# joe5saia/Hmc.jl

Hardware: NVIDIA B200
Metric: HMM state-steps/sec (windows x chains x T per Gibbs sweep) (higher is better)
Workload: dtype f32

## Files before the change

### hmc.jl_b200/csrc/hmcgpu.cu

```cuda
#include "../../include/hmcgpu.h"
#include "gibbs_wide_kernel.cuh"
#include "gibbs_scan_kernel.cuh"
#include "gibbs_seg_kernel.cuh"
#include "diagnostics.cuh"

#include <algorithm>
#include <chrono>
#include <condition_variable>
#include <cmath>
#include <cstdarg>
#include <cstdio>
#include <cstdlib>
#include <cstring>
#include <exception>
#include <map>
#include <memory>
#include <mutex>
#include <new>
#include <numeric>
#include <optional>
#include <string>
#include <thread>
#include <vector>

// ... 1083 lines not shown
    totS[slot] = w < 0 ? R(0) : (R)wi[w].totS;
    totQ[slot] = w < 0 ? R(0) : (R)wi[w].totQ;
    if (cntM) {
        totSm[slot] = w < 0 ? R(0) : (R)wi[w].totSm;
        totQm[slot] = w < 0 ? R(0) : (R)wi[w].totQm;
        totM[slot] = w < 0 ? 0 : (int)wi[w].totM;
    }
}

template <typename R>
__global__ void sigw_kernel(long long y_len, int S, const unsigned char* __restrict__ sig, double kappa,
                            unsigned char* __restrict__ mask_tm, R* __restrict__ out) {
    const long long i = blockIdx.x * (long long)blockDim.x + threadIdx.x;
    if (i >= y_len * S) return;
    const long long t = i / S;
    const int s = (int)(i % S);
    const bool f = sig && sig[(long long)s * y_len + t];
    if (mask_tm) mask_tm[i] = f ? 1 : 0;
    out[i] = f ? (R)(-1.0 / (1.0 + kappa)) : R(1);
}

template <typename R>
__global__ void __launch_bounds__(256) y_layout_kernel(long long y_len, int n_series, const double* __restrict__ in, R* __restrict__ yr) {
    __shared__ double tile[32][33];
    const long long s0 = (long long)blockIdx.x * 32, t0 = (long long)blockIdx.y * 32;
    const int tx = threadIdx.x & 31, ty = threadIdx.x >> 5;
#pragma unroll
    for (int j = ty; j < 32; j += 8) {
        const long long sidx = s0 + j, t = t0 + tx;
        if (sidx < n_series && t < y_len) tile[j][tx] = in[sidx * y_len + t];
    }
    __syncthreads();
#pragma unroll
    for (int j = ty; j < 32; j += 8) {
        const long long t = t0 + j, sidx = s0 + tx;
        if (sidx < n_series && t < y_len) yr[t * n_series + sidx] = (R)tile[tx][j];
    }
}

__global__ void summary_finish_kernel(long long n_elems, int F, double n, int has_loglik, const double* __restrict__ sum,
                                      const double* __restrict__ sumsq, double* __restrict__ mean, double* __restrict__ var) {
    const long long i = blockIdx.x * (long long)blockDim.x + threadIdx.x;
    if (i >= n_elems) return;
    const bool zero = !has_loglik && (int)(i % F) == F - 1;
    const double m = sum[i] / n;
    mean[i] = zero ? 0.0 : m;
    var[i] = zero ? 0.0 : fmax(0.0, __dsub_rn(sumsq[i] / n, __dmul_rn(m, m)));
}

template <typename R>
__global__ void yfut_kernel(int n_slots, int n_h, const int* __restrict__ slot_win, const double* __restrict__ yfut_w, R* __restrict__ out) {
    const int slot = blockIdx.x * blockDim.x + threadIdx.x;
    if (slot >= n_slots) return;
    const int w = slot_win[slot];
    for (int j = 0; j < n_h; ++j) out[(size_t)j * n_slots + slot] = w < 0 ? R(0) : (R)yfut_w[(size_t)w * n_h + j];
}

template <typename R>
__global__ void gather_draws_kernel(int K, int n_h, int n_slots, int chunk, int n_i, long long draw0, long long nrun, int n_chains,
                                    const int* __restrict__ slot_win, const int* __restrict__ slot_chain,
                                    const R* __restrict__ out, double* mu, double* sig2, double* A, double* pie, double* fc, double* ll) {
    const int i = blockIdx.y * blockDim.y + threadIdx.y;
    const int slot = blockIdx.x * blockDim.x + threadIdx.x;
    if (slot >= n_slots || i >= n_i) return;
    const int w = slot_win[slot];
    if (w < 0) return;
    const long long Rr = (long long)n_chains * nrun;
    const long long d = (long long)slot_chain[slot] * nrun + draw0 + i;
    const size_t cs = (size_t)chunk * n_slots;
    const R* o = out + (size_t)i * n_slots + slot;
    int f = 0;
    for (int k = 0; k < K; ++k, ++f) if (mu) mu[(size_t)w * Rr * K + (size_t)k * Rr + d] = (double)o[f * cs];
    for (int k = 0; k < K; ++k, ++f) if (sig2) sig2[(size_t)w * Rr * K + (size_t)k * Rr + d] = (double)o[f * cs];
    for (int k = 0; k < K * K; ++k, ++f) if (A) A[(size_t)w * Rr * K * K + (size_t)k * Rr + d] = (double)o[f * cs];
    for (int k = 0; k < K; ++k, ++f) if (pie) pie[(size_t)w * Rr * K + (size_t)k * Rr + d] = (double)o[f * cs];
    for (int k = 0; k < 2 * n_h; ++k, ++f) if (fc) fc[(size_t)w * Rr * 2 * n_h + (size_t)k * Rr + d] = (double)o[f * cs];
    if (ll) ll[(size_t)w * Rr + d] = (double)o[f * cs];
}

template <typename R>
__global__ void __launch_bounds__(128) summary_accum_kernel(int F, int n_slots, int chunk, int n_i, int n_chains,
                                                            const int* __restrict__ win_slot0, const R* __restrict__ out,
                                                            double* __restrict__ sum, double* __restrict__ sumsq) {
    __shared__ double sh[128];
    const int w = blockIdx.x, f = blockIdx.y;
    const int s0 = win_slot0[w];
    double a = 0.0, b = 0.0;
    const long long n = (long long)n_chains * n_i;
    for (long long j = threadIdx.x; j < n; j += blockDim.x) {
        const int cidx = (int)(j % n_chains), i = (int)(j / n_chains);
        const double v = (double)out[((size_t)f * chunk + i) * n_slots + s0 + cidx];
        a += v; b += v * v;
    }
    auto add = [](double x, double y2) { return x + y2; };
    a = block_reduce<double>(a, sh, add);
    b = block_reduce<double>(b, sh, add);
    if (threadIdx.x == 0) { sum[(size_t)w * F + f] += a; sumsq[(size_t)w * F + f] += b; }
}

template <typename R>
__global__ void tile_reduce_kernel(int K, int ncols, int n_chains, const int* __restrict__ win_slot0, const int* __restrict__ wT,
                                   const long long* __restrict__ warp_pi_off, const int* __restrict__ warp_T,
                                   const long long* __restrict__ win_off, R* __restrict__ acc_tile, double* __restrict__ win_sum) {
    const int w = blockIdx.x;
    const int N = wT[w];
    const int s0 = win_slot0[w];
    double* dst = win_sum + win_off[w] / K * ncols;
    for (int e = threadIdx.x; e < N * ncols; e += blockDim.x) {
        const int t = e / ncols, k = e % ncols;
        double acc = 0.0;
        for (int cidx = 0; cidx < n_chains; ++cidx) {
            const int slot = s0 + cidx;
            const int row = t + (warp_T[slot >> 5] - N);
            R* p = acc_tile + warp_pi_off[slot >> 5] / K * ncols + (size_t)(row * ncols + k) * 32 + (slot & 31);
            acc += (double)*p;
            *p = R(0);
        }
        dst[(size_t)k * N + t] += acc;
    }
}

struct SweepChoice {
    SweepKernel kernel = SweepKernel::thread;
    int seg_lanes = 0;
    int n_long = 0;
    int sweeps_per_launch = 16;
    int seg_threads = 128;
};

struct hmcgpu_plan {
    hmcgpu_ctx* ctx = nullptr;
    int K = 0, n_chains = 0, n_windows = 0, n_h = 0, precision = 32;
    long long burnin = 0, nrun = 0;
    unsigned flags = 0;
    unsigned long long seed = 0;
    int F = 0;
    std::vector<int> wT;
    std::vector<int> order;
    std::vector<long long> pib_off;
    long long pib_total = 0;
    long long state_steps = 0;
    int n_slots = 0, n_warps = 0, n_tasks = 0, chunk = 0, max_T = 0;
    GibbsArgs args{};
    DevBuf yr, wbase, wTd, wi, slot_win, slot_chain, T, ybase, warp_T, warp_pi_off, pi, pacc, facc, cnt, trans, Sd, Qd,
        events, cshift, xi, xi_user, chain_id, out, yfut_w, yfut, win_slot0, win_pib_off, totS, totQ, slot_pi_off;
    DevBuf sigmask, sigmask_tm, sigw, sbase, wsbase, wbase_init, X0, x0_off, cntM, Sm, Qm, totSm, totQm, totM;
    bool sig = false;
    Tuning tuning;
    SweepChoice sw;
    DevBuf yin;
    DevBuf warp_T_long, warp_pi_off_long;
    struct Group { int task0, stride, n_tasks, lanes; bool long_class; };
    std::vector<Group> groups;
    int n_groups = 1, n_bufs = 1;
    std::vector<cudaStream_t> gstreams;
    std::vector<cudaEvent_t> pool_events;
    std::vector<cudaEvent_t> timing_events;
    double launch_ms_sum = 0.0;
    DevBuf d_mu, d_sig2, d_A, d_pie, d_fc, d_ll, d_sum, d_sumsq, d_pibsum, d_fcsum;
    DevBuf dg_P, dg_S1, dg_head, dg_ring, dg_mean, dg_var, dg_gsum;
    DevBuf d_diag;
    unsigned long long seg_fallbacks[2] = {0, 0};
    cudaEvent_t ev0 = nullptr, ev1 = nullptr, evk0 = nullptr, evk1 = nullptr;
    double gpu_ms = 0.0, sweep_ms = 0.0;
    long long n_launches = 0, n_sweep_launches = 0, h2d = 0, d2h = 0;
    bool ran = false;
    ~hmcgpu_plan() {
        for (auto s2 : gstreams) cudaStreamDestroy(s2);
        for (auto e : pool_events) cudaEventDestroy(e);
        for (auto e : timing_events) cudaEventDestroy(e);
        if (ev0) cudaEventDestroy(ev0);
        if (ev1) cudaEventDestroy(ev1);
        if (evk0) cudaEventDestroy(evk0);
        if (evk1) cudaEventDestroy(evk1);
    }
};

static int validate_problem(hmcgpu_ctx* ctx, const hmcgpu_problem* p, const Tuning& t) {
    if (!ctx) return HMCGPU_ERR_ARG;
    if (!p) return fail(ctx, HMCGPU_ERR_ARG, "problem is NULL");
    if (!p->y || p->y_len < 2 || p->n_series < 1) return fail(ctx, HMCGPU_ERR_ARG, "empty series");
    if (p->n_windows < 1 || !p->win_start || !p->win_end) return fail(ctx, HMCGPU_ERR_ARG, "no windows");
    if (!k_supported(p->K)) return fail(ctx, HMCGPU_ERR_UNSUPPORTED, "K=%d not supported (2..32)", p->K);
    if (!k_thread_sweep(p->K, t) && (p->flags & HMCGPU_FLAG_SMOOTHED_MEAN))
        return fail(ctx, HMCGPU_ERR_UNSUPPORTED, "smoothed means are only implemented for K <= 8 (thread-per-chain kernels)");
    if (p->K > 4 && (p->flags & (HMCGPU_FLAG_SMOOTHED_MEAN | HMCGPU_FLAG_FILTERED_MEAN)) && p->n_h > 0) {
        const size_t b = p->precision / 8;
        const size_t need = (size_t)(p->K * b + 8 + 15) / 16 * 16 * p->K * 128 + b * 4 * 3 * 4 * p->K * 32 + b * (size_t)p->n_h * (p->K + 1) * 128;
        if (need > 200 * 1024)
            return fail(ctx, HMCGPU_ERR_UNSUPPORTED, "K=%d with %d in-sample forecast horizons needs %zu KB of shared memory per block: use fewer horizons", p->K, p->n_h, need / 1024);
    }
    if (p->flags & HMCGPU_FLAG_FILTERED_MEAN) {
        if (!k_thread_sweep(p->K, t)) return fail(ctx, HMCGPU_ERR_UNSUPPORTED, "filtered means are only implemented for K <= 8");
        if (p->flags & HMCGPU_FLAG_SMOOTHED_MEAN) return fail(ctx, HMCGPU_ERR_UNSUPPORTED, "HMCGPU_FLAG_FILTERED_MEAN and HMCGPU_FLAG_SMOOTHED_MEAN share their output arrays: one per call");
        if (p->is_signal || p->pi_row_back != 0) return fail(ctx, HMCGPU_ERR_UNSUPPORTED, "is_signal / pi_row_back cannot be combined with HMCGPU_FLAG_FILTERED_MEAN");
    }
    if (p->n_chains < 1) return fail(ctx, HMCGPU_ERR_ARG, "n_chains < 1");
    if ((long long)p->n_windows * p->n_chains > 0x7fffffffLL - 64)
        return fail(ctx, HMCGPU_ERR_UNSUPPORTED, "n_windows * n_chains = %lld exceeds 2^31 - 65 chains per call", (long long)p->n_windows * p->n_chains);
    if (p->burnin < 0 || p->nrun < 1) return fail(ctx, HMCGPU_ERR_ARG, "burnin < 0 or nrun < 1");
    if (p->burnin + p->nrun > 0xffffffffLL) return fail(ctx, HMCGPU_ERR_ARG, "more than 2^32 sweeps");
    if ((p->flags & HMCGPU_FLAG_DIAGNOSTICS) && p->nrun < 4) return fail(ctx, HMCGPU_ERR_ARG, "HMCGPU_FLAG_DIAGNOSTICS needs nrun >= 4 (two sequences of >= 2 draws per chain)");
    if (p->precision != 32 && p->precision != 64) return fail(ctx, HMCGPU_ERR_ARG, "precision must be 32 or 64");
    if (p->n_h < 0 || p->n_h > kMaxH || (p->n_h > 0 && !p->horizons)) return fail(ctx, HMCGPU_ERR_ARG, "0 <= n_h <= %d", kMaxH);
    if (p->is_signal || p->pi_row_back != 0) {
        if (!k_thread(p->K)) return fail(ctx, HMCGPU_ERR_UNSUPPORTED, "is_signal / pi_row_back are only implemented for K <= 4");
        if (p->flags & HMCGPU_FLAG_SMOOTHED_MEAN) return fail(ctx, HMCGPU_ERR_UNSUPPORTED, "is_signal / pi_row_back cannot be combined with HMCGPU_FLAG_SMOOTHED_MEAN");
        if (p->is_signal && !(p->kappa >= 0.0)) return fail(ctx, HMCGPU_ERR_ARG, "kappa must be >= 0 with is_signal");
        if (p->pi_row_back < 0) return fail(ctx, HMCGPU_ERR_ARG, "pi_row_back < 0");
    }
    for (int j = 0; j < p->n_h; ++j)
        if (p->horizons[j] < 0 || p->horizons[j] > kMaxHorizon) return fail(ctx, HMCGPU_ERR_ARG, "horizons must be in 0..%d", kMaxHorizon);
    for (int i = 0; i < p->K; ++i) {
        if ((p->alpha && !(p->alpha[i] > 0.0)) || (p->nu && !(p->nu[i] > 0.0)) || (p->beta0 && !(p->beta0[i] > 0.0)) || (p->beta && !(p->beta[i] > 0.0)))
            return fail(ctx, HMCGPU_ERR_ARG, "alpha, nu, beta0 and beta must be > 0 (state %d)", i + 1);
        if (p->xi && !std::isfinite(p->xi[i])) return fail(ctx, HMCGPU_ERR_ARG, "xi[%d] is not finite", i);
    }
    for (int w = 0; w < p->n_windows; ++w) {
        const long long wid = p->win_id ? (long long)p->win_id[w] : (long long)w;
        if (wid < 0 || (wid + 1) * (long long)p->n_chains > 0x100000000LL)
            return fail(ctx, HMCGPU_ERR_ARG, "window %d: win_id %lld with %d chains per window leaves the 32-bit chain-id range", w, wid, p->n_chains);
        const long long s = p->win_start[w], e = p->win_end[w];
        if (s < 1 || e > p->y_len || e - s + 1 < 2) return fail(ctx, HMCGPU_ERR_ARG, "window %d: [%lld,%lld] outside 1..%lld or shorter than 2", w, s, e, (long long)p->y_len);
        if (p->win_series && (p->win_series[w] < 0 || p->win_series[w] >= p->n_series)) return fail(ctx, HMCGPU_ERR_ARG, "window %d: bad series index", w);
        if (p->win_init_series && (p->win_init_series[w] < 0 || p->win_init_series[w] >= p->n_series)) return fail(ctx, HMCGPU_ERR_ARG, "window %d: bad init series index", w);
        if (p->pi_row_back >= e - s + 1) return fail(ctx, HMCGPU_ERR_ARG, "window %d: pi_row_back %d >= window length", w, p->pi_row_back);
    }
    if (p->X0) {
        size_t off = 0;
        for (int w = 0; w < p->n_windows; ++w) {
            const long long n = (long long)p->win_end[w] - p->win_start[w] + 1;
            for (long long i = 0; i < n; ++i)
                if (p->X0[off + i] < 1 || p->X0[off + i] > p->K) return fail(ctx, HMCGPU_ERR_ARG, "X0: state %lld of window %d is outside 1..%d", (long long)p->X0[off + i], w, p->K);
            off += (size_t)n;
        }
    }
    return 0;
}

static int scan_max_T_of(int precision, int K) { DISPATCH_K(K, return precision == 32 ? scan_max_T<float, KK>() : scan_max_T<double, KK>()); return 0; }
static long long seg_max_T_of(int K, int lanes) { DISPATCH_K(K, return seg_max_T<KK>(lanes)); return 0; }

static int choose_sweep(hmcgpu_ctx* ctx, const hmcgpu_problem* p, const std::vector<int>& wT, const std::vector<int>& order,
                        const Tuning& t, SweepChoice& c) {
    const int K = p->K, nw = p->n_windows, nc = p->n_chains, max_T = wT[order[0]];
    const bool sig = p->is_signal != nullptr || p->pi_row_back != 0;
    const bool acc_mean = p->flags & (HMCGPU_FLAG_SMOOTHED_MEAN | HMCGPU_FLAG_FILTERED_MEAN);
    const long long n_real = (long long)nw * nc;
    const long long full = (long long)ctx->sm_count * 16 * 32;
    c = SweepChoice{};
    if (!k_thread_sweep(K, t)) c.kernel = SweepKernel::lane;
// ... 213 lines not shown
    CU(ctx, pl->cnt.alloc((size_t)K * n_slots * sizeof(int)));
    CU(ctx, pl->trans.alloc((size_t)K * K * n_slots * sizeof(int)));
    CU(ctx, pl->Sd.alloc((size_t)K * n_slots * sizeof(R)));
    CU(ctx, pl->Qd.alloc((size_t)K * n_slots * sizeof(R)));
    CU(ctx, pl->events.alloc((size_t)n_slots * sizeof(int)));
    CU(ctx, pl->cshift.alloc((size_t)n_slots * sizeof(R)));
    CU(ctx, pl->xi.alloc((size_t)K * n_slots * sizeof(R)));
    CU(ctx, pl->totS.alloc((size_t)n_slots * sizeof(R)));
    CU(ctx, pl->totQ.alloc((size_t)n_slots * sizeof(R)));
    CU(ctx, pl->out.alloc(per_draw * (size_t)chunk * pl->n_bufs));
    CU(ctx, pl->yfut.alloc((size_t)std::max(1, p->n_h) * n_slots * sizeof(R)));
    const size_t Rr = (size_t)nc * p->nrun;
    if (p->flags & HMCGPU_FLAG_DRAWS) {
        CU(ctx, pl->d_mu.alloc((size_t)nw * Rr * K * sizeof(double)));
        CU(ctx, pl->d_sig2.alloc((size_t)nw * Rr * K * sizeof(double)));
        CU(ctx, pl->d_A.alloc((size_t)nw * Rr * K * K * sizeof(double)));
        CU(ctx, pl->d_pie.alloc((size_t)nw * Rr * K * sizeof(double)));
        if (p->n_h > 0) CU(ctx, pl->d_fc.alloc((size_t)nw * Rr * 2 * p->n_h * sizeof(double)));
        if (p->flags & HMCGPU_FLAG_LOGLIK) CU(ctx, pl->d_ll.alloc((size_t)nw * Rr * sizeof(double)));
    }
    if (p->flags & HMCGPU_FLAG_SUMMARY) {
        CU(ctx, pl->d_sum.alloc((size_t)nw * pl->F * sizeof(double)));
        CU(ctx, pl->d_sumsq.alloc((size_t)nw * pl->F * sizeof(double)));
    }
    if (p->flags & HMCGPU_FLAG_DIAGNOSTICS) {
        const size_t n_sf = (size_t)pl->F * n_slots, nwf = (size_t)nw * pl->F;
        CU(ctx, pl->dg_P.alloc(n_sf * kDiagLags * sizeof(double)));
        CU(ctx, pl->dg_S1.alloc(n_sf * sizeof(double)));
        CU(ctx, pl->dg_head.alloc(n_sf * kDiagLags * sizeof(R)));
        CU(ctx, pl->dg_ring.alloc(n_sf * kDiagLags * sizeof(R)));
        CU(ctx, pl->dg_mean.alloc(nwf * 2 * nc * sizeof(double)));
        CU(ctx, pl->dg_var.alloc(nwf * 2 * nc * sizeof(double)));
        CU(ctx, pl->dg_gsum.alloc(nwf * kDiagLags * sizeof(double)));
    }
    if (p->flags & kAccMean) {
        CU(ctx, pl->pacc.alloc((size_t)lay.pi_elems * sizeof(R)));
        if (p->n_h > 0) {
            CU(ctx, pl->facc.alloc((size_t)lay.pi_elems / K * p->n_h * sizeof(R)));
            CU(ctx, pl->d_fcsum.alloc((size_t)pib_total / K * p->n_h * sizeof(double)));
        }
        CU(ctx, pl->d_pibsum.alloc((size_t)pib_total * sizeof(double)));
    }
    const size_t smem = (size_t)pl->max_T;
    if (smem > 200 * 1024) return fail(ctx, HMCGPU_ERR_UNSUPPORTED, "window longer than %d observations", 200 * 1024);
    if (smem > 48 * 1024) CU(ctx, cudaFuncSetAttribute(window_init_kernel, cudaFuncAttributeMaxDynamicSharedMemorySize, (int)smem));
    window_init_kernel<<<nw, 256, smem, st>>>(K, yin.as<double>(), 1, pl->wbase.as<long long>(), pl->wbase_init.as<long long>(),
                                              pl->wTd.as<int>(), p->is_signal ? pl->sigmask_tm.as<unsigned char>() : nullptr,
                                              pl->wsbase.as<long long>(), sld, pl->X0.as<long long>(),
                                              pl->x0_off.as<long long>(), pl->wi.as<WinInit>());
    CU(ctx, cudaGetLastError());
    tr.sync_mark(st, "  tables, allocations, window statistics");
    yfut_kernel<R><<<grid_for(n_slots, 128), 128, 0, st>>>(n_slots, p->n_h, pl->slot_win.as<int>(), pl->yfut_w.as<double>(), pl->yfut.as<R>());
    CU(ctx, cudaGetLastError());

    GibbsArgs& a = pl->args;
    a.n_slots = n_slots; a.T = pl->T.as<int>(); a.ybase = pl->ybase.as<long long>(); a.yld = nser; a.y = pl->yr.p;
    a.warp_T = pl->warp_T.as<int>(); a.warp_pi_off = pl->warp_pi_off.as<long long>(); a.pi = pl->pi.p; a.pib_acc = pl->pacc.p; a.fc_acc = pl->facc.p;
    a.cnt = pl->cnt.as<int>(); a.trans = pl->trans.as<int>(); a.Sd = pl->Sd.p; a.Qd = pl->Qd.p; a.events = pl->events.as<int>();
    a.cshift = pl->cshift.p; a.xi = pl->xi.p; a.totS = pl->totS.p; a.totQ = pl->totQ.p; a.n_warps = n_warps;
    for (int i = 0; i < 32; ++i) {
        a.alpha[i] = (p->alpha && i < K) ? p->alpha[i] : 1.0;
        a.nu[i] = (p->nu && i < K) ? p->nu[i] : 1.0;
        a.beta0[i] = (p->beta0 && i < K) ? p->beta0[i] : 1.0;
        a.beta[i] = (p->beta && i < K) ? p->beta[i] : 2.0;
    }
    a.k0 = (unsigned)p->seed; a.k1 = (unsigned)(p->seed >> 32); a.chain_id = pl->chain_id.as<unsigned>();
    a.burnin = p->burnin; a.out = pl->out.p; a.chunk = pl->chunk; a.n_h = p->n_h;
    for (int j = 0; j < p->n_h; ++j) { a.h_sorted[j] = p->horizons[hs[j]]; a.h_slot[j] = hs[j]; }
    a.yfut = pl->yfut.p; a.flags = p->flags;
    a.sigw = pl->sigw.p; a.sbase = pl->sbase.as<long long>(); a.sld = sld; a.cntM = pl->cntM.as<int>(); a.Sm = pl->Sm.p; a.Qm = pl->Qm.p; a.totSm = pl->totSm.p; a.totQm = pl->totQm.p;
    a.totM = pl->totM.as<int>(); a.kappa = p->kappa; a.pi_back = p->pi_row_back;
    a.y_sm_elems = (y_in_smem<R>() && nser == 1 && K <= 4 && pl->sw.kernel == SweepKernel::thread && (size_t)p->y_len * sizeof(R) <= (size_t)kYSmemMaxBytes &&
                    pl->tuning.y_smem) ? (int)p->y_len : 0;
    a.all_signal = 0;
    if (p->is_signal) {
        const size_t nm = (size_t)p->y_len * sld;
        size_t ones = 0;
        for (size_t q = 0; q < nm; ++q) ones += p->is_signal[q] != 0;
        a.all_signal = ones == nm;
    }
    a.seg_warm = pl->tuning.seg_warm; a.seg_barriers = pl->tuning.seg_barriers;
    if (pl->sw.kernel == SweepKernel::seg) CU(ctx, pl->d_diag.alloc(2 * sizeof(unsigned long long)));
    a.diag = pl->d_diag.as<unsigned long long>();
    for (int g = 0; g < pl->n_groups; ++g) {
        cudaStream_t s2;
        CU(ctx, cudaStreamCreateWithFlags(&s2, cudaStreamNonBlocking));
        pl->gstreams.push_back(s2);
    }
    CU(ctx, cudaEventCreate(&pl->ev0)); CU(ctx, cudaEventCreate(&pl->ev1));
    CU(ctx, cudaEventCreate(&pl->evk0)); CU(ctx, cudaEventCreate(&pl->evk1));
    tr.mark("  tables, allocations, init");
    CU(ctx, cudaStreamSynchronize(st));
    tr.mark("  stream drained");
    pl->yin.release();
    return HMCGPU_OK;
}

template <typename R, int K>
static int plan_run_t(hmcgpu_plan* pl) {
    hmcgpu_ctx* ctx = pl->ctx;
    cudaStream_t st = ctx->stream;
    const int ns = pl->n_slots, G = pl->n_groups;
    const int L = pl->sw.sweeps_per_launch;
    const int Kr = pl->K;
    pl->n_launches = 0; pl->n_sweep_launches = 0; pl->sweep_ms = 0.0;
    size_t ev_used = 0;
    auto new_event = [&](cudaEvent_t* e) -> cudaError_t {
        if (ev_used == pl->pool_events.size()) {
            cudaEvent_t x;
            cudaError_t rc = cudaEventCreateWithFlags(&x, cudaEventDisableTiming);
            if (rc != cudaSuccess) return rc;
            pl->pool_events.push_back(x);
        }
        *e = pl->pool_events[ev_used++];
        return cudaSuccess;
    };
    CU(ctx, cudaEventRecord(pl->ev0, st));
    chain_init_kernel<R><<<grid_for(ns, 128), 128, 0, st>>>(Kr, ns, pl->slot_win.as<int>(), pl->wi.as<WinInit>(),
                                                             pl->xi_user.as<double>(), pl->cnt.as<int>(), pl->trans.as<int>(),
                                                             pl->Sd.as<R>(), pl->Qd.as<R>(), pl->cshift.as<R>(), pl->xi.as<R>(),
                                                             pl->totS.as<R>(), pl->totQ.as<R>(), pl->events.as<int>(),
                                                             pl->cntM.as<int>(), pl->Sm.as<R>(), pl->Qm.as<R>(), pl->totSm.as<R>(),
                                                             pl->totQm.as<R>(), pl->totM.as<int>());
    CU(ctx, cudaGetLastError());
    ++pl->n_launches;
    if (pl->d_diag.p) CU(ctx, cudaMemsetAsync(pl->d_diag.p, 0, 2 * sizeof(unsigned long long), st));
    if (pl->d_sum.p) { CU(ctx, cudaMemsetAsync(pl->d_sum.p, 0, pl->d_sum.bytes, st)); CU(ctx, cudaMemsetAsync(pl->d_sumsq.p, 0, pl->d_sumsq.bytes, st)); }
    if (pl->pacc.p) { CU(ctx, cudaMemsetAsync(pl->pacc.p, 0, pl->pacc.bytes, st)); CU(ctx, cudaMemsetAsync(pl->d_pibsum.p, 0, pl->d_pibsum.bytes, st)); }
    if (pl->facc.p) { CU(ctx, cudaMemsetAsync(pl->facc.p, 0, pl->facc.bytes, st)); CU(ctx, cudaMemsetAsync(pl->d_fcsum.p, 0, pl->d_fcsum.bytes, st)); }
    cudaEvent_t ev_init;
    CU(ctx, new_event(&ev_init));
    CU(ctx, cudaEventRecord(ev_init, st));
    CU(ctx, cudaEventRecord(pl->evk0, st));
    for (int g = 0; g < G; ++g) CU(ctx, cudaStreamWaitEvent(pl->gstreams[g], ev_init, 0));
    size_t tev_used = 0;
    auto timing_event = [&](cudaEvent_t* e) -> cudaError_t {
        if (tev_used == pl->timing_events.size()) {
            cudaEvent_t x;
            cudaError_t rc = cudaEventCreate(&x);
            if (rc != cudaSuccess) return rc;
            pl->timing_events.push_back(x);
        }
        *e = pl->timing_events[tev_used++];
        return cudaSuccess;
    };
    std::vector<cudaEvent_t> gend(G, nullptr);
    for (int g = 0; g < G; ++g) CU(ctx, timing_event(&gend[g]));
    std::vector<std::pair<cudaEvent_t, cudaEvent_t>> launch_pairs;

    const GibbsLaunch cfg{pl->flags, pl->max_T, ctx->sm_count, pl->n_h, pl->sig};
    const long long S = pl->burnin + pl->nrun;
    const long long n_chunks = (pl->nrun + pl->chunk - 1) / pl->chunk;
    const size_t buf_elems = (size_t)pl->F * pl->chunk * ns;
    std::vector<long long> next(G, 0);
    std::vector<cudaEvent_t> post_done(n_chunks, nullptr);
    std::vector<std::vector<cudaEvent_t>> chunk_done(n_chunks, std::vector<cudaEvent_t>(G, nullptr));
    long long posted = 0;
    auto enqueue_post = [&](long long k) -> int {
        for (int g = 0; g < G; ++g) CU(ctx, cudaStreamWaitEvent(st, chunk_done[k][g], 0));
        const long long d0 = k * pl->chunk;
        const int n = (int)std::min<long long>(pl->chunk, pl->nrun - d0);
        const R* buf = pl->out.as<R>() + (size_t)(k % pl->n_bufs) * buf_elems;
        if (pl->flags & HMCGPU_FLAG_DRAWS) {
            dim3 blk(32, 8), grd(grid_for(ns, 32), grid_for(n, 8));
            gather_draws_kernel<R><<<grd, blk, 0, st>>>(Kr, pl->n_h, ns, pl->chunk, n, d0, pl->nrun, pl->n_chains, pl->slot_win.as<int>(),
                                                         pl->slot_chain.as<int>(), buf, pl->d_mu.as<double>(), pl->d_sig2.as<double>(),
                                                         pl->d_A.as<double>(), pl->d_pie.as<double>(), pl->d_fc.as<double>(), pl->d_ll.as<double>());
            CU(ctx, cudaGetLastError());
            ++pl->n_launches;
        }
        if (pl->flags & HMCGPU_FLAG_SUMMARY) {
            dim3 grd(pl->n_windows, pl->F);
            summary_accum_kernel<R><<<grd, 128, 0, st>>>(pl->F, ns, pl->chunk, n, pl->n_chains, pl->win_slot0.as<int>(), buf,
                                                         pl->d_sum.as<double>(), pl->d_sumsq.as<double>());
            CU(ctx, cudaGetLastError());
            ++pl->n_launches;
        }
        if (pl->flags & HMCGPU_FLAG_DIAGNOSTICS) {
            const long long nh = pl->nrun / 2, h2 = pl->nrun - nh;
            const int Fd = (pl->flags & HMCGPU_FLAG_LOGLIK) ? pl->F : pl->F - 1;
            const DiagState<R> ds{pl->dg_P.as<double>(), pl->dg_S1.as<double>(), pl->dg_head.as<R>(), pl->dg_ring.as<R>(), (long long)pl->F * ns};
            auto sequence = [&](long long lo, long long hi, long long seq0, long long seq_end, int half) -> int {
                if (lo >= hi) return 0;
                diag_accum_kernel<R><<<dim3(ns / 32, Fd), dim3(32, 32), 0, st>>>(ns, pl->chunk, (int)(lo - d0), (int)(hi - lo), lo - seq0, buf, ds);
                CU(ctx, cudaGetLastError());
                ++pl->n_launches;
                if (hi == seq_end) {
                    diag_half_kernel<R><<<dim3(pl->n_windows, Fd), kDiagLags, 0, st>>>(pl->F, ns, pl->n_chains, nh, half, pl->win_slot0.as<int>(), ds,
                                                                                       pl->dg_mean.as<double>(), pl->dg_var.as<double>(), pl->dg_gsum.as<double>());
                    CU(ctx, cudaGetLastError());
                    ++pl->n_launches;
                }
                return 0;
            };
            TRY(sequence(d0, std::min<long long>(d0 + n, nh), 0, nh, 0));
            TRY(sequence(std::max(d0, h2), d0 + n, h2, pl->nrun, 1));
        }
        if (pl->flags & (HMCGPU_FLAG_SMOOTHED_MEAN | HMCGPU_FLAG_FILTERED_MEAN)) {
            tile_reduce_kernel<R><<<pl->n_windows, 256, 0, st>>>(Kr, Kr, pl->n_chains, pl->win_slot0.as<int>(), pl->wTd.as<int>(),
                                                                 pl->warp_pi_off.as<long long>(), pl->warp_T.as<int>(), pl->win_pib_off.as<long long>(),
                                                                 pl->pacc.as<R>(), pl->d_pibsum.as<double>());
            CU(ctx, cudaGetLastError());
            ++pl->n_launches;
            if (pl->facc.p) {
                tile_reduce_kernel<R><<<pl->n_windows, 256, 0, st>>>(Kr, pl->n_h, pl->n_chains, pl->win_slot0.as<int>(), pl->wTd.as<int>(),
                                                                     pl->warp_pi_off.as<long long>(), pl->warp_T.as<int>(), pl->win_pib_off.as<long long>(),
                                                                     pl->facc.as<R>(), pl->d_fcsum.as<double>());
                CU(ctx, cudaGetLastError());
                ++pl->n_launches;
            }
        }
        CU(ctx, new_event(&post_done[k]));
        CU(ctx, cudaEventRecord(post_done[k], st));
        return 0;
    };
    GibbsArgs a = pl->args;
    auto enqueue_one = [&](const int g, const long long round) -> int {
            const long long s0 = next[g];
            if (s0 >= S) return 1;
            if (s0 >= pl->burnin && (s0 - pl->burnin) % pl->chunk == 0) {
                const long long k0 = (s0 - pl->burnin) / pl->chunk;
                if (k0 >= pl->n_bufs && post_done[k0 - pl->n_bufs] == nullptr) return 1;
            }
            long long n = (round == 0 && G > 1) ? std::max<long long>(1, (long long)L * (g + 1) / G) : L;
            long long limit = S;
            if (s0 < pl->burnin) limit = pl->burnin;
            else limit = pl->burnin + std::min<long long>(pl->nrun, ((s0 - pl->burnin) / pl->chunk + 1) * pl->chunk);
            n = std::min(n, limit - s0);
            cudaStream_t gs = pl->gstreams[g];
            long long k = -1;
            if (s0 >= pl->burnin) {
                k = (s0 - pl->burnin) / pl->chunk;
                if ((s0 - pl->burnin) % pl->chunk == 0 && k >= pl->n_bufs) CU(ctx, cudaStreamWaitEvent(gs, post_done[k - pl->n_bufs], 0));
                a.draw0 = k * pl->chunk;
                a.out = pl->out.as<R>() + (size_t)(k % pl->n_bufs) * buf_elems;
            } else {
                a.draw0 = 0;
                a.out = pl->out.p;
            }
            a.sweep0 = s0; a.n_sweeps = (int)n;
            const hmcgpu_plan::Group& grp = pl->groups[g];
            a.task0 = grp.task0; a.task_stride = grp.stride; a.n_tasks = grp.n_tasks;
            a.warp_T = grp.long_class ? pl->warp_T_long.as<int>() : pl->warp_T.as<int>();
            a.warp_pi_off = grp.long_class ? pl->warp_pi_off_long.as<long long>() : pl->warp_pi_off.as<long long>();
            cudaEvent_t lt0 = nullptr, lt1 = nullptr;
            if (pl->tuning.launch_timing) { CU(ctx, timing_event(&lt0)); CU(ctx, timing_event(&lt1)); CU(ctx, cudaEventRecord(lt0, gs)); }
            if constexpr (K == 0) {
                CU(ctx, (launch_gibbs_wide<R>(cfg, a, pl->K, pl->slot_pi_off.as<long long>(), gs)));
            } else if constexpr (K <= 4) {
                switch (pl->sw.kernel) {
                    case SweepKernel::scan: CU(ctx, (launch_gibbs_scan<R, K>(cfg, a, gs))); break;
                    case SweepKernel::seg: CU(ctx, (launch_gibbs_seg<R, K>(cfg, a, grp.lanes, pl->sw.seg_threads, gs))); break;
                    default: CU(ctx, (launch_gibbs<R, K>(cfg, a, gs)));
                }
            } else {
                CU(ctx, (launch_gibbs<R, K>(cfg, a, gs)));
            }
            if (pl->tuning.launch_timing) { CU(ctx, cudaEventRecord(lt1, gs)); launch_pairs.emplace_back(lt0, lt1); }
            ++pl->n_launches; ++pl->n_sweep_launches;
            next[g] = s0 + n;
            if (next[g] >= S) CU(ctx, cudaEventRecord(gend[g], gs));
            if (k >= 0 && next[g] == pl->burnin + std::min<long long>(pl->nrun, (k + 1) * pl->chunk)) {
                CU(ctx, new_event(&chunk_done[k][g]));
                CU(ctx, cudaEventRecord(chunk_done[k][g], gs));
            }
            while (posted < n_chunks) {
                bool ready = true;
                for (int g2 = 0; g2 < G; ++g2) ready = ready && chunk_done[posted][g2] != nullptr;
                if (!ready) break;
                TRY(enqueue_post(posted));
                ++posted;
            }
            return 0;
    };
    PhaseTrace trr;
    bool more = true;
    for (long long round = 0; more; ++round) {
        more = false;
        std::vector<int> gorder(G);
        std::iota(gorder.begin(), gorder.end(), 0);
        std::stable_sort(gorder.begin(), gorder.end(), [&](int x, int y2) { return next[x] < next[y2]; });
        for (int g : gorder) {
            if (next[g] >= S) continue;
            more = true;
            const int rc = enqueue_one(g, round);
            if (rc < 0) return rc;
        }
    }
    CU(ctx, cudaEventRecord(pl->ev1, st));
    trr.mark("    launches enqueued");
    CU(ctx, cudaEventSynchronize(pl->ev1));
    trr.mark("    device drained");
    for (int g = 0; g < G; ++g) CU(ctx, cudaStreamSynchronize(pl->gstreams[g]));
    float ms = 0.f;
    CU(ctx, cudaEventElapsedTime(&ms, pl->ev0, pl->ev1));
    pl->gpu_ms = ms;
    pl->sweep_ms = 0.0;
    for (int g = 0; g < G; ++g) {
        float t = 0.f;
        CU(ctx, cudaEventElapsedTime(&t, pl->evk0, gend[g]));
        pl->sweep_ms = std::max(pl->sweep_ms, (double)t);
    }
    pl->launch_ms_sum = 0.0;
    for (auto& pr : launch_pairs) {
        float t = 0.f;
        CU(ctx, cudaEventElapsedTime(&t, pr.first, pr.second));
        pl->launch_ms_sum += t;
    }
    if (pl->d_diag.p) {
        CU(ctx, cudaMemcpy(pl->seg_fallbacks, pl->d_diag.p, 2 * sizeof(unsigned long long), cudaMemcpyDeviceToHost));
        if (pl->tuning.verbose) {
            const double cs = (double)pl->n_windows * pl->n_chains * (double)S;
            if (pl->sw.n_long) fprintf(stderr, "[hmcgpu] segment kernel: the %d longest of %d windows with 8 lanes per chain\n", pl->sw.n_long, pl->n_windows);
            fprintf(stderr, "[hmcgpu] segment kernel (%d lanes per chain, warm-up %d): %llu of %.0f chain-sweeps used the exact entering vectors; "
                            "%.2f speculative groups of 4 steps per chain-sweep\n",
                    pl->sw.seg_lanes, pl->args.seg_warm, pl->seg_fallbacks[0], cs, (double)pl->seg_fallbacks[1] / cs);
        }
    }
    pl->ran = true;
    return HMCGPU_OK;
}

static int plan_create_impl(hmcgpu_ctx* ctx, const hmcgpu_problem* p, hmcgpu_plan** out) {
    const Tuning t = read_tuning();
    TRY(validate_problem(ctx, p, t));
    CU(ctx, cudaSetDevice(ctx->device));
    tl_pool = ctx->pool;
    std::unique_ptr<hmcgpu_plan> pl(new hmcgpu_plan());
    pl->ctx = ctx;
    pl->tuning = t;
    int rc = (p->precision == 32) ? plan_build<float>(pl.get(), p) : plan_build<double>(pl.get(), p);
    if (rc != 0) {
        cudaStreamSynchronize(ctx->stream);
        cudaGetLastError();
        return rc;
    }
    *out = pl.release();
    return HMCGPU_OK;
}

extern "C" int hmcgpu_plan_create(hmcgpu_ctx* ctx, const hmcgpu_problem* p, hmcgpu_plan** out) {
    if (!out) return fail(ctx, HMCGPU_ERR_ARG, "out is NULL");
    *out = nullptr;
    GUARD(ctx, plan_create_impl(ctx, p, out));
}

static int plan_run_impl(hmcgpu_plan* pl) {
    hmcgpu_ctx* ctx = pl->ctx;
    CU(ctx, cudaSetDevice(ctx->device));
    int rc = HMCGPU_ERR_UNSUPPORTED;
    DISPATCH_RUN(pl, rc);
    return rc;
}

extern "C" int hmcgpu_plan_run(hmcgpu_plan* pl) {
    if (!pl) return HMCGPU_ERR_ARG;
    GUARD(pl->ctx, plan_run_impl(pl));
}

static int plan_fetch_impl(hmcgpu_plan* pl, hmcgpu_result* r);
extern "C" int hmcgpu_plan_fetch(hmcgpu_plan* pl, hmcgpu_result* r) {
    if (!pl || !r) return HMCGPU_ERR_ARG;
    GUARD(pl->ctx, plan_fetch_impl(pl, r));
}

static int plan_fetch_impl(hmcgpu_plan* pl, hmcgpu_result* r) {
    hmcgpu_ctx* ctx = pl->ctx;
    if (!pl->ran) return fail(ctx, HMCGPU_ERR_ARG, "plan_fetch before plan_run");
    CU(ctx, cudaSetDevice(ctx->device));
    cudaStream_t st = ctx->stream;
    const int K = pl->K, nw = pl->n_windows;
    const size_t Rr = (size_t)pl->n_chains * pl->nrun;
    long long d2h = 0;
    auto down = [&](void* host, const DevBuf& b, size_t bytes) -> cudaError_t {
        if (!host || !b.p) return cudaSuccess;
        d2h += (long long)bytes;
        return cudaMemcpyAsync(host, b.p, bytes, cudaMemcpyDeviceToHost, st);
    };
    if ((r->mu || r->sigma2 || r->A || r->pi_end || r->forecasts || r->loglik) && !(pl->flags & HMCGPU_FLAG_DRAWS))
        return fail(ctx, HMCGPU_ERR_ARG, "per-draw outputs requested without HMCGPU_FLAG_DRAWS");
    if ((r->summary_mean || r->summary_var) && !(pl->flags & HMCGPU_FLAG_SUMMARY))
        return fail(ctx, HMCGPU_ERR_ARG, "summary requested without HMCGPU_FLAG_SUMMARY");
    if ((r->pib_mean || r->insample_forecast_mean) && !(pl->flags & (HMCGPU_FLAG_SMOOTHED_MEAN | HMCGPU_FLAG_FILTERED_MEAN)))
        return fail(ctx, HMCGPU_ERR_ARG, "pib_mean / insample_forecast_mean requested without HMCGPU_FLAG_SMOOTHED_MEAN or HMCGPU_FLAG_FILTERED_MEAN");
    if (r->loglik && !(pl->flags & HMCGPU_FLAG_LOGLIK)) return fail(ctx, HMCGPU_ERR_ARG, "loglik requested without HMCGPU_FLAG_LOGLIK");
    const bool diag = (pl->flags & HMCGPU_FLAG_DIAGNOSTICS) && (r->rhat || r->ess || r->ess_lag);
    CU(ctx, down(r->mu, pl->d_mu, nw * Rr * K * sizeof(double)));
    CU(ctx, down(r->sigma2, pl->d_sig2, nw * Rr * K * sizeof(double)));
    CU(ctx, down(r->A, pl->d_A, nw * Rr * K * K * sizeof(double)));
    CU(ctx, down(r->pi_end, pl->d_pie, nw * Rr * K * sizeof(double)));
    CU(ctx, down(r->forecasts, pl->d_fc, nw * Rr * 2 * pl->n_h * sizeof(double)));
    CU(ctx, down(r->loglik, pl->d_ll, nw * Rr * sizeof(double)));
    std::vector<double> pibsum, fcsum;
    std::vector<int> ev(pl->n_slots);
    DevBuf d_mean, d_var;
    if (r->summary_mean || r->summary_var) {
        const long long ne = (long long)nw * pl->F;
        CU(ctx, d_mean.alloc((size_t)ne * sizeof(double)));
        CU(ctx, d_var.alloc((size_t)ne * sizeof(double)));
        summary_finish_kernel<<<grid_for(ne, 256), 256, 0, st>>>(ne, pl->F, (double)Rr, (pl->flags & HMCGPU_FLAG_LOGLIK) ? 1 : 0,
                                                                 pl->d_sum.as<double>(), pl->d_sumsq.as<double>(), d_mean.as<double>(), d_var.as<double>());
        CU(ctx, cudaGetLastError());
        CU(ctx, down(r->summary_mean, d_mean, (size_t)ne * sizeof(double)));
        CU(ctx, down(r->summary_var, d_var, (size_t)ne * sizeof(double)));
    }
    DevBuf d_rhat, d_ess, d_lag;
    if (diag) {
        const long long ne = (long long)nw * pl->F;
        CU(ctx, d_rhat.alloc((size_t)ne * sizeof(double)));
        CU(ctx, d_ess.alloc((size_t)ne * sizeof(double)));
        CU(ctx, d_lag.alloc((size_t)ne * sizeof(int)));
        diag_finish_kernel<<<grid_for(ne, 128), 128, 0, st>>>(ne, pl->F, pl->n_chains, pl->nrun / 2, (pl->flags & HMCGPU_FLAG_LOGLIK) ? 1 : 0,
                                                              pl->dg_mean.as<double>(), pl->dg_var.as<double>(), pl->dg_gsum.as<double>(),
                                                              d_rhat.as<double>(), d_ess.as<double>(), d_lag.as<int>());
        CU(ctx, cudaGetLastError());
        CU(ctx, down(r->rhat, d_rhat, (size_t)ne * sizeof(double)));
        CU(ctx, down(r->ess, d_ess, (size_t)ne * sizeof(double)));
        CU(ctx, down(r->ess_lag, d_lag, (size_t)ne * sizeof(int)));
    }
    if (r->pib_mean) { pibsum.resize((size_t)pl->pib_total); CU(ctx, down(pibsum.data(), pl->d_pibsum, pibsum.size() * sizeof(double))); }
    if (r->insample_forecast_mean && pl->d_fcsum.p) {
        fcsum.resize((size_t)pl->pib_total / K * pl->n_h);
        CU(ctx, down(fcsum.data(), pl->d_fcsum, fcsum.size() * sizeof(double)));
    }
    CU(ctx, down(ev.data(), pl->events, ev.size() * sizeof(int)));
    CU(ctx, cudaStreamSynchronize(st));
    const double n = (double)Rr;
    for (size_t i = 0; i < pibsum.size(); ++i) r->pib_mean[i] = pibsum[i] / n;
    for (size_t i = 0; i < fcsum.size(); ++i) r->insample_forecast_mean[i] = fcsum[i] / n;
    std::vector<int> slot_win(pl->n_slots), slot_chain(pl->n_slots);
    int bad = 0;
    for (int j = 0; j < nw; ++j) {
        const int w = pl->order[j];
        for (int c = 0; c < pl->n_chains; ++c) {
            const int e = ev[(size_t)j * pl->n_chains + c];
            if (r->status) r->status[(size_t)w * pl->n_chains + c] = e;
            bad += e != 0;
        }
    }
    r->gpu_ms = pl->gpu_ms; r->sweep_kernel_ms = pl->sweep_ms; r->n_launches = pl->n_launches;
    r->n_sweep_launches = pl->n_sweep_launches; r->h2d_bytes = pl->h2d; r->d2h_bytes = d2h; r->state_steps = pl->state_steps;
    r->sweep_launch_ms_sum = pl->launch_ms_sum;
    r->sweep_kernel = (int32_t)pl->sw.kernel;
    r->n_tasks = pl->n_tasks;
    return bad;
}

extern "C" void hmcgpu_plan_destroy(hmcgpu_plan* pl) {
    if (!pl) return;
    cudaSetDevice(pl->ctx->device);
    cudaStreamSynchronize(pl->ctx->stream);
    for (auto s2 : pl->gstreams) cudaStreamSynchronize(s2);
    delete pl;
}

extern "C" int hmcgpu_estimate(hmcgpu_ctx* ctx, const hmcgpu_problem* p, hmcgpu_result* r) {
    if (!r) return fail(ctx, HMCGPU_ERR_ARG, "result is NULL");
    hmcgpu_plan* pl = nullptr;
    PhaseTrace tr;
    TRY(hmcgpu_plan_create(ctx, p, &pl));
    tr.mark("plan_create (upload, init)");
    int rc = hmcgpu_plan_run(pl);
    tr.mark("plan_run (all sweeps)");
    if (rc == 0) rc = hmcgpu_plan_fetch(pl, r);
    tr.mark("plan_fetch (download)");
    hmcgpu_plan_destroy(pl);
    tr.mark("plan_destroy");
    return rc;
}

static int estimate_multi_impl(const int* devices, int n_dev, const hmcgpu_problem* p, hmcgpu_result* r);
extern "C" int hmcgpu_estimate_multi(const int* devices, int n_dev, const hmcgpu_problem* p, hmcgpu_result* r) {
    if (!devices || n_dev < 1 || !p || !r) return fail(nullptr, HMCGPU_ERR_ARG, "bad arguments");
    GUARD(nullptr, estimate_multi_impl(devices, n_dev, p, r));
}

static int estimate_multi_impl(const int* devices, int n_dev, const hmcgpu_problem* p, hmcgpu_result* r) {
    if (p->n_windows < 1 || !p->win_start || !p->win_end) return fail(nullptr, HMCGPU_ERR_ARG, "no windows");
    const int nw = p->n_windows, K = p->K, nh = p->n_h;
    std::vector<int> ord(nw);
    std::iota(ord.begin(), ord.end(), 0);
    auto Tw = [&](int w) { return p->win_end[w] - p->win_start[w] + 1; };
    std::stable_sort(ord.begin(), ord.end(), [&](int a, int b) { return Tw(a) > Tw(b); });
    std::vector<std::vector<int>> shard(n_dev);
    std::vector<long long> load(n_dev, 0);
    for (int w : ord) {
        const int d = (int)(std::min_element(load.begin(), load.end()) - load.begin());
        shard[d].push_back(w);
        load[d] += Tw(w);
    }
    const size_t Rr = (size_t)p->n_chains * p->nrun;
    const int F = 3 * K + K * K + 2 * nh + 1;
    std::vector<long long> pib_off(nw);
    long long acc = 0;
    for (int w = 0; w < nw; ++w) { pib_off[w] = acc; acc += (long long)Tw(w) * K; }
    std::vector<int> rcs(n_dev, 0);
    std::vector<std::string> errs(n_dev);
    std::vector<hmcgpu_result> parts(n_dev);
    std::vector<std::thread> th;
    for (int d = 0; d < n_dev; ++d) {
        th.emplace_back([&, d]() {
          hmcgpu_ctx* ctx = nullptr;
          try {
            const std::vector<int>& ws = shard[d];
            const int n = (int)ws.size();
            memset(&parts[d], 0, sizeof(hmcgpu_result));
            if (n == 0) return;
            int rc = hmcgpu_ctx_create(devices[d], &ctx);
            if (rc != 0) { rcs[d] = rc; errs[d] = hmcgpu_last_error(nullptr); return; }
            std::vector<int32_t> ser(n), iser(n), st(n), en(n);
            std::vector<int64_t> id(n), x0;
            size_t pibn = 0;
            for (int j = 0; j < n; ++j) {
                const int w = ws[j];
                ser[j] = p->win_series ? p->win_series[w] : 0; st[j] = p->win_start[w]; en[j] = p->win_end[w];
                iser[j] = p->win_init_series ? p->win_init_series[w] : ser[j];
                id[j] = p->win_id ? p->win_id[w] : w;
                pibn += (size_t)Tw(w) * K;
                if (p->X0) x0.insert(x0.end(), p->X0 + pib_off[w] / K, p->X0 + pib_off[w] / K + Tw(w));
            }
            hmcgpu_problem q = *p;
            q.n_windows = n; q.win_series = ser.data(); q.win_start = st.data(); q.win_end = en.data(); q.win_id = id.data();
            if (p->win_init_series) q.win_init_series = iser.data();
            if (p->X0) q.X0 = x0.data();
            std::vector<double> mu, s2, A, pe, fc, ll, sm, sv, pb, ifc, rh, es;
            std::vector<int32_t> status, el;
            const bool diag = (p->flags & HMCGPU_FLAG_DIAGNOSTICS) != 0;
            hmcgpu_result& o = parts[d];
            if (r->mu) { mu.resize(n * Rr * K); o.mu = mu.data(); }
            if (r->sigma2) { s2.resize(n * Rr * K); o.sigma2 = s2.data(); }
            if (r->A) { A.resize(n * Rr * K * K); o.A = A.data(); }
            if (r->pi_end) { pe.resize(n * Rr * K); o.pi_end = pe.data(); }
            if (r->forecasts) { fc.resize(n * Rr * 2 * nh); o.forecasts = fc.data(); }
            if (r->loglik) { ll.resize(n * Rr); o.loglik = ll.data(); }
            if (r->summary_mean) { sm.resize((size_t)n * F); o.summary_mean = sm.data(); }
// ... 55 lines not shown
```

Baseline: 227.4 billion.

## Run post-processing on low-priority stream and batch summary accumulation loads

Moves all per-chunk post-processing kernels (draw gather, summary, diagnostics, tile reduce) from the main context stream to a dedicated low-priority stream, and gives the Gibbs sweep group streams high priority. This lets post-processing overlap with sweeps instead of serializing on the main stream. The summary accumulation kernel is also rewritten to replace per-element div/mod indexing with incremental offsets and software-pipelined batched loads. The end-of-run event now waits on the last post event, which assumes n_chunks > 0 and that its event is non-null.

```diff
diff --git a/hmc.jl_b200/csrc/hmcgpu.cu b/hmc.jl_b200/csrc/hmcgpu.cu
--- a/hmc.jl_b200/csrc/hmcgpu.cu
+++ b/hmc.jl_b200/csrc/hmcgpu.cu
@@ -1189,15 +1189,46 @@
 __global__ void __launch_bounds__(128) summary_accum_kernel(int F, int n_slots, int chunk, int n_i, int n_chains,
                                                             const int* __restrict__ win_slot0, const R* __restrict__ out,
                                                             double* __restrict__ sum, double* __restrict__ sumsq) {
+    constexpr int kBatch = 8;
     __shared__ double sh[128];
     const int w = blockIdx.x, f = blockIdx.y;
-    const int s0 = win_slot0[w];
+    const int t = threadIdx.x, nt = blockDim.x;
+    const int n = n_chains * n_i;
+    const int cnt = t < n ? (n - t + nt - 1) / nt : 0;
+    const int dc = nt % n_chains;
+    const unsigned step = (unsigned)(nt / n_chains) * n_slots + dc, carry = n_slots - n_chains;
+    const R* const plane = out + (size_t)f * chunk * n_slots + win_slot0[w];
+    int c = t % n_chains;
+    unsigned off = (unsigned)(t / n_chains) * n_slots + c;
+    auto advance = [&] {
+        off += step;
+        c += dc;
+        if (c >= n_chains) { c -= n_chains; off += carry; }
+    };
     double a = 0.0, b = 0.0;
-    const long long n = (long long)n_chains * n_i;
-    for (long long j = threadIdx.x; j < n; j += blockDim.x) {
-        const int cidx = (int)(j % n_chains), i = (int)(j / n_chains);
-        const double v = (double)out[((size_t)f * chunk + i) * n_slots + s0 + cidx];
-        a += v; b += v * v;
+    int e = 0;
+    R v[kBatch];
+    auto load = [&](R* dst) {
+#pragma unroll
+        for (int u = 0; u < kBatch; ++u) { dst[u] = plane[off]; advance(); }
+    };
+    auto accumulate = [&] {
+#pragma unroll
+        for (int u = 0; u < kBatch; ++u) { const double x = (double)v[u]; a += x; b += x * x; }
+    };
+    if (cnt >= kBatch) load(v);
+    for (; e + 2 * kBatch <= cnt; e += kBatch) {
+        R nv[kBatch];
+        load(nv);
+        accumulate();
+#pragma unroll
+        for (int u = 0; u < kBatch; ++u) v[u] = nv[u];
+    }
+    if (e + kBatch <= cnt) { accumulate(); e += kBatch; }
+    for (; e < cnt; ++e) {
+        const double x = (double)plane[off];
+        advance();
+        a += x; b += x * x;
     }
     auto add = [](double x, double y2) { return x + y2; };
     a = block_reduce<double>(a, sh, add);
@@ -1261,6 +1292,7 @@
     std::vector<Group> groups;
     int n_groups = 1, n_bufs = 1;
     std::vector<cudaStream_t> gstreams;
+    cudaStream_t post_stream = nullptr;
     std::vector<cudaEvent_t> pool_events;
     std::vector<cudaEvent_t> timing_events;
     double launch_ms_sum = 0.0;
@@ -1274,6 +1306,7 @@
     bool ran = false;
     ~hmcgpu_plan() {
         for (auto s2 : gstreams) cudaStreamDestroy(s2);
+        if (post_stream) cudaStreamDestroy(post_stream);
         for (auto e : pool_events) cudaEventDestroy(e);
         for (auto e : timing_events) cudaEventDestroy(e);
         if (ev0) cudaEventDestroy(ev0);
@@ -1653,11 +1686,14 @@
     a.seg_warm = pl->tuning.seg_warm; a.seg_barriers = pl->tuning.seg_barriers;
     if (pl->sw.kernel == SweepKernel::seg) CU(ctx, pl->d_diag.alloc(2 * sizeof(unsigned long long)));
     a.diag = pl->d_diag.as<unsigned long long>();
+    int prio_low = 0, prio_high = 0;
+    CU(ctx, cudaDeviceGetStreamPriorityRange(&prio_low, &prio_high));
     for (int g = 0; g < pl->n_groups; ++g) {
         cudaStream_t s2;
-        CU(ctx, cudaStreamCreateWithFlags(&s2, cudaStreamNonBlocking));
+        CU(ctx, cudaStreamCreateWithPriority(&s2, cudaStreamNonBlocking, prio_high));
         pl->gstreams.push_back(s2);
     }
+    CU(ctx, cudaStreamCreateWithPriority(&pl->post_stream, cudaStreamNonBlocking, prio_low));
     CU(ctx, cudaEventCreate(&pl->ev0)); CU(ctx, cudaEventCreate(&pl->ev1));
     CU(ctx, cudaEventCreate(&pl->evk0)); CU(ctx, cudaEventCreate(&pl->evk1));
     tr.mark("  tables, allocations, init");
@@ -1670,7 +1706,7 @@
 template <typename R, int K>
 static int plan_run_t(hmcgpu_plan* pl) {
     hmcgpu_ctx* ctx = pl->ctx;
-    cudaStream_t st = ctx->stream;
+    cudaStream_t st = ctx->stream, ps = pl->post_stream;
     const int ns = pl->n_slots, G = pl->n_groups;
     const int L = pl->sw.sweeps_per_launch;
     const int Kr = pl->K;
@@ -1728,13 +1764,13 @@
     std::vector<std::vector<cudaEvent_t>> chunk_done(n_chunks, std::vector<cudaEvent_t>(G, nullptr));
     long long posted = 0;
     auto enqueue_post = [&](long long k) -> int {
-        for (int g = 0; g < G; ++g) CU(ctx, cudaStreamWaitEvent(st, chunk_done[k][g], 0));
+        for (int g = 0; g < G; ++g) CU(ctx, cudaStreamWaitEvent(ps, chunk_done[k][g], 0));
         const long long d0 = k * pl->chunk;
         const int n = (int)std::min<long long>(pl->chunk, pl->nrun - d0);
         const R* buf = pl->out.as<R>() + (size_t)(k % pl->n_bufs) * buf_elems;
         if (pl->flags & HMCGPU_FLAG_DRAWS) {
             dim3 blk(32, 8), grd(grid_for(ns, 32), grid_for(n, 8));
-            gather_draws_kernel<R><<<grd, blk, 0, st>>>(Kr, pl->n_h, ns, pl->chunk, n, d0, pl->nrun, pl->n_chains, pl->slot_win.as<int>(),
+            gather_draws_kernel<R><<<grd, blk, 0, ps>>>(Kr, pl->n_h, ns, pl->chunk, n, d0, pl->nrun, pl->n_chains, pl->slot_win.as<int>(),
                                                          pl->slot_chain.as<int>(), buf, pl->d_mu.as<double>(), pl->d_sig2.as<double>(),
                                                          pl->d_A.as<double>(), pl->d_pie.as<double>(), pl->d_fc.as<double>(), pl->d_ll.as<double>());
             CU(ctx, cudaGetLastError());
@@ -1742,7 +1778,7 @@
         }
         if (pl->flags & HMCGPU_FLAG_SUMMARY) {
             dim3 grd(pl->n_windows, pl->F);
-            summary_accum_kernel<R><<<grd, 128, 0, st>>>(pl->F, ns, pl->chunk, n, pl->n_chains, pl->win_slot0.as<int>(), buf,
+            summary_accum_kernel<R><<<grd, 128, 0, ps>>>(pl->F, ns, pl->chunk, n, pl->n_chains, pl->win_slot0.as<int>(), buf,
                                                          pl->d_sum.as<double>(), pl->d_sumsq.as<double>());
             CU(ctx, cudaGetLastError());
             ++pl->n_launches;
@@ -1753,11 +1789,11 @@
             const DiagState<R> ds{pl->dg_P.as<double>(), pl->dg_S1.as<double>(), pl->dg_head.as<R>(), pl->dg_ring.as<R>(), (long long)pl->F * ns};
             auto sequence = [&](long long lo, long long hi, long long seq0, long long seq_end, int half) -> int {
                 if (lo >= hi) return 0;
-                diag_accum_kernel<R><<<dim3(ns / 32, Fd), dim3(32, 32), 0, st>>>(ns, pl->chunk, (int)(lo - d0), (int)(hi - lo), lo - seq0, buf, ds);
+                diag_accum_kernel<R><<<dim3(ns / 32, Fd), dim3(32, 32), 0, ps>>>(ns, pl->chunk, (int)(lo - d0), (int)(hi - lo), lo - seq0, buf, ds);
                 CU(ctx, cudaGetLastError());
                 ++pl->n_launches;
                 if (hi == seq_end) {
-                    diag_half_kernel<R><<<dim3(pl->n_windows, Fd), kDiagLags, 0, st>>>(pl->F, ns, pl->n_chains, nh, half, pl->win_slot0.as<int>(), ds,
+                    diag_half_kernel<R><<<dim3(pl->n_windows, Fd), kDiagLags, 0, ps>>>(pl->F, ns, pl->n_chains, nh, half, pl->win_slot0.as<int>(), ds,
                                                                                        pl->dg_mean.as<double>(), pl->dg_var.as<double>(), pl->dg_gsum.as<double>());
                     CU(ctx, cudaGetLastError());
                     ++pl->n_launches;
@@ -1768,13 +1804,13 @@
             TRY(sequence(std::max(d0, h2), d0 + n, h2, pl->nrun, 1));
         }
         if (pl->flags & (HMCGPU_FLAG_SMOOTHED_MEAN | HMCGPU_FLAG_FILTERED_MEAN)) {
-            tile_reduce_kernel<R><<<pl->n_windows, 256, 0, st>>>(Kr, Kr, pl->n_chains, pl->win_slot0.as<int>(), pl->wTd.as<int>(),
+            tile_reduce_kernel<R><<<pl->n_windows, 256, 0, ps>>>(Kr, Kr, pl->n_chains, pl->win_slot0.as<int>(), pl->wTd.as<int>(),
                                                                  pl->warp_pi_off.as<long long>(), pl->warp_T.as<int>(), pl->win_pib_off.as<long long>(),
                                                                  pl->pacc.as<R>(), pl->d_pibsum.as<double>());
             CU(ctx, cudaGetLastError());
             ++pl->n_launches;
             if (pl->facc.p) {
-                tile_reduce_kernel<R><<<pl->n_windows, 256, 0, st>>>(Kr, pl->n_h, pl->n_chains, pl->win_slot0.as<int>(), pl->wTd.as<int>(),
+                tile_reduce_kernel<R><<<pl->n_windows, 256, 0, ps>>>(Kr, pl->n_h, pl->n_chains, pl->win_slot0.as<int>(), pl->wTd.as<int>(),
                                                                      pl->warp_pi_off.as<long long>(), pl->warp_T.as<int>(), pl->win_pib_off.as<long long>(),
                                                                      pl->facc.as<R>(), pl->d_fcsum.as<double>());
                 CU(ctx, cudaGetLastError());
@@ -1782,7 +1818,7 @@
             }
         }
         CU(ctx, new_event(&post_done[k]));
-        CU(ctx, cudaEventRecord(post_done[k], st));
+        CU(ctx, cudaEventRecord(post_done[k], ps));
         return 0;
     };
     GibbsArgs a = pl->args;
@@ -1858,6 +1894,7 @@
             if (rc < 0) return rc;
         }
     }
+    CU(ctx, cudaStreamWaitEvent(st, post_done[n_chunks - 1], 0));
     CU(ctx, cudaEventRecord(pl->ev1, st));
     trr.mark("    launches enqueued");
     CU(ctx, cudaEventSynchronize(pl->ev1));
@@ -2022,6 +2059,7 @@
     cudaSetDevice(pl->ctx->device);
     cudaStreamSynchronize(pl->ctx->stream);
     for (auto s2 : pl->gstreams) cudaStreamSynchronize(s2);
+    if (pl->post_stream) cudaStreamSynchronize(pl->post_stream);
     delete pl;
 }
 
```

Measured after the change: 231.0 billion, median of 6. 1.02x the previous value.
